# amit154154/HyperscaleES_T2I

Hardware: AMD Instinct MI355X
Metric: ES member-evals/sec (whole node) Sana-Sprint 1.6B pop=64; % HBM/MFMA roofline (higher is better)
Workload: dtype bf16; 1 GPU; sana_sprint_1.6b_onestep_1024px_es_epoch; pop_per_gpu=8, pop_total=8, images_per_member=16, prompts_per_gen=4, batches_per_gen=4, resolution_px=1024, egg_rank=1, lora_r=2, lora_alpha=8, theta_D=1515456, antithetic=True, promptnorm=True, reward=PickScore(CLIP-H/14)+CLIP-B/32, parallelism=member-shard x1 (S all-gather)

## Files before the change

### hyperscalees_t2i_amd/_lib.py

```python
from __future__ import annotations

import ctypes as C
import hashlib
import os
import re
from pathlib import Path

_PKG = Path(__file__).resolve().parent
LIB_PATH = _PKG / "_build" / "libeggroll.so"
HEADER = _PKG.parent / "include" / "eggroll.h"
from .build_ext import SOURCES

SOURCE_FILES = [_PKG / "csrc" / n for n in SOURCES] + sorted((_PKG / "csrc").glob("*.h")) + [HEADER]

i32, i64, u32, u64, f32 = C.c_int32, C.c_int64, C.c_uint32, C.c_uint64, C.c_float
vp = C.c_void_p

SIGNATURES = {
    "eggroll_version": (C.c_char_p, []),
    "eggroll_last_error": (C.c_char_p, []),
    "eggroll_noise_factors": (C.c_int, [u64, i64, i64, i64, i64, vp, vp]),
    "eggroll_philox_words": (C.c_int, [u64, i64, i64, vp, vp]),
    "eggroll_perturb": (C.c_int, [vp, vp, i64, i64, vp, vp, i64, i64, i32, i32, i32, i64, i64, f32, vp, i64, vp]),
    "eggroll_perturb_seeded": (C.c_int, [u64, vp, vp, vp, i64, i64, i32, i32, i32, i64, i64, f32, vp, i64, vp]),
# ... 5 lines not shown
    "eggroll_update_seeded": (C.c_int, [u64, vp, vp, vp, i32, i32, vp, vp, i64, i64, i32, f32, f32, f32, vp, vp, vp]),
    "eggroll_lora_linear_pop": (C.c_int, [vp, i64, vp, i64, vp, vp, i64, i64, i64, i32, f32, i64, i64, i64, i64, vp,
                                          i64, vp, vp]),
    "eggroll_lora_gemm": (C.c_int, [vp, i64, vp, i64, vp, vp, vp, i64, i64, i32, f32, i64, i64, i64, i64, vp, i64, vp]),
    "eggroll_lora_gemm_sel": (C.c_int, [vp, i64, vp, i64, vp, vp, vp, i64, i64, i32, f32, i64, i64, i64, i64, vp, i64,
                                        i32, vp]),
    "eggroll_lora_linear_pop_sel": (C.c_int, [vp, i64, vp, i64, vp, vp, i64, i64, i64, i32, f32, i64, i64, i64, i64,
                                              vp, i64, vp, i32, vp]),
    "eggroll_lora_workspace_bytes": (i64, [i64, i64, i32, i64]),
    "eggroll_lora_project": (C.c_int, [vp, i64, vp, i64, i64, i32, i64, i64, i64, vp, vp]),
    "eggroll_lora_project_multi": (C.c_int, [vp, i64, vp, i64, vp, i32, i32, i64, i64, i64, vp, vp]),
    "eggroll_lora_delta_f32": (C.c_int, [vp, i64, vp, i64, vp, i64, i32, f32, i64, i64, i64, i64, vp, i64, vp]),
    "eggroll_dwconv_nhwc": (C.c_int, [vp, vp, vp, i64, i64, i64, i64, i32, i32, i32, vp, vp]),
    "eggroll_rownorm": (C.c_int, [vp, i64, i64, f32, i32, vp, vp, vp, vp, i64, i64, i32, vp, vp, vp]),
    "eggroll_gated_residual": (C.c_int, [vp, vp, vp, i64, i64, i64, i64, vp]),
    "eggroll_rownorm_ex": (C.c_int, [vp, i32, i64, i64, f32, i32, vp, vp, vp, vp, i64, i32, i64, i32, vp, i32, vp, i32,
                                     vp, vp]),
    "eggroll_subpixel_shortcut_f32": (C.c_int, [vp, vp, vp, vp, vp, i64, i64, i64, i64, i64, vp]),
    "eggroll_gated_residual_f32": (C.c_int, [vp, vp, vp, i32, i64, i64, i64, i64, vp, vp]),
    "eggroll_scm_step": (C.c_int, [vp, i64, vp, i32, vp, i64, i64, f32, f32, f32, f32, f32, f32, f32, f32, f32, i32, vp,
                                   vp, vp, vp]),
    "eggroll_resid_layernorm": (C.c_int, [vp, i64, vp, i64, i64, i64, f32, vp, vp, vp, vp]),
    "eggroll_dwconv_pw_nhwc": (C.c_int, [vp, vp, vp, i64, i64, i64, i64, i32, vp, vp]),
    "eggroll_dwconv_nhwc_sel": (C.c_int, [vp, vp, vp, i64, i64, i64, i64, i32, i32, i32, vp, i32, vp]),
    "eggroll_qk_norm_rope": (C.c_int, [vp, i64, i64, i32, i32, f32, vp, vp, vp, i64, vp]),
    "eggroll_qk_norm_rope_kv": (C.c_int, [vp, i64, i64, i32, i32, f32, vp, vp, vp, i64, vp, vp, i64, i64, i64, i64, vp, i64, vp, vp]),
    "eggroll_qk_l2norm_kv": (C.c_int, [vp, i64, vp, i64, vp, i64, i64, i32, i32, f32, vp, vp, vp, i64, i64, i64, i64, vp]),
    "eggroll_group_norm_workspace_bytes": (C.c_int64, [i64, i64, i32, i32]),
    "eggroll_group_norm_nhwc": (C.c_int, [vp, i64, i64, i32, i32, f32, vp, vp, i32, vp, vp, vp]),
    "eggroll_flash_attention": (C.c_int, [vp, i64, i64, vp, i64, i64, vp, i64, i64, i64, i64, i64, i64, i64, f32, vp, i64, i64, vp]),
    "eggroll_flash_attention_sel": (C.c_int, [vp, i64, i64, vp, i64, i64, vp, i64, i64, i64, i64, i64, i64, i64, f32, vp, i64, i64, i32, vp]),
    "eggroll_dwconv_nhwc_ex": (C.c_int, [vp, vp, vp, i64, i64, i64, i64, i32, i32, i32, vp, i64, i32, vp]),
    "eggroll_dwconv_pw_nhwc_sel": (C.c_int, [vp, vp, vp, i64, i64, i64, i64, i32, vp, i32, vp]),
    "eggroll_upshortcut_add": (C.c_int, [vp, vp, i64, i64, i64, i64, i64, vp]),
    "eggroll_subpixel_shortcut": (C.c_int, [vp, vp, vp, vp, i64, i64, i64, i64, i64, vp]),
    "eggroll_bias_act": (C.c_int, [vp, vp, i64, i64, i32, vp]),
    "eggroll_conv3x3_nhwc": (C.c_int, [vp, vp, vp, i64, i64, i64, i64, i64, i32, i32, vp, vp]),
    "eggroll_conv_nhwc": (C.c_int, [vp, vp, vp, i64, i64, i64, i64, i64, i32, i32, i32, vp, vp]),
    "eggroll_conv3x3_rmsnorm_nhwc": (C.c_int, [vp, vp, vp, i64, i64, i64, i64, i64, i32, C.c_float, vp, vp, vp, vp,
                                               vp]),
    "eggroll_conv_nhwc_sel": (C.c_int, [vp, vp, vp, i64, i64, i64, i64, i64, i32, i32, i32, vp, i32, vp]),
    "eggroll_conv2x2_subpixel_nhwc": (C.c_int, [vp, vp, vp, vp, i32, i64, i64, i64, i64, i64, vp, vp, vp]),
    "eggroll_conv3x3_rmsnorm_nhwc_sel": (C.c_int, [vp, vp, vp, i64, i64, i64, i64, i64, i32, C.c_float, vp, vp, vp,
                                                   vp, i32, vp]),
    "eggroll_dcae_head": (C.c_int, [vp, i64, i64, i64, i64, f32, vp, vp, vp, vp, vp, vp]),
    "eggroll_linear_attention_workspace_bytes": (i64, [i64, i64, i64]),
    "eggroll_linear_attention": (C.c_int, [vp, vp, vp, i64, i64, i64, i64, i64, i32, vp, i64, vp, vp]),
    "eggroll_lora_expand": (C.c_int, [vp, vp, i64, i64, i32, f32, i64, i64, i64, vp, i64, vp]),
    "eggroll_lora_linear_pop_epi": (C.c_int, [vp, i64, vp, i64, vp, vp, i64, i64, i64, i32, f32, i64, i64, i64, i64,
                                              vp, i64, vp, i32, vp, i64, vp, i64, i64, vp]),
    "eggroll_lora_linear_pop_epi_sel": (C.c_int, [vp, i64, vp, i64, vp, vp, i64, i64, i64, i32, f32, i64, i64, i64,
                                                  i64, vp, i64, vp, i32, vp, i64, vp, i64, i64, i32, vp]),
    "eggroll_lora_gemm_epi_sel": (C.c_int, [vp, i64, vp, i64, vp, vp, vp, i64, i64, i32, f32, i64, i64, i64, i64,
                                            vp, i64, i32, vp, i64, vp, i64, i64, i32, vp]),
    "eggroll_cross_attention": (C.c_int, [vp, i64, vp, vp, i64, vp, vp, i64, i64, i64, i64, i64, i64, f32, vp, i64,
                                         vp]),
    "eggroll_cross_attention_sel": (C.c_int, [vp, i64, vp, vp, i64, vp, vp, i64, i64, i64, i64, i64, i64, f32, vp,
                                             i64, i32, vp]),
    "eggroll_clip_preprocess": (C.c_int, [vp, i64, i64, i64, i64, i64, i64, i64, i32, vp, vp, i32, i32, i64, i64,
                                          i64, vp, vp, vp, vp, vp]),
    "eggroll_clip_preprocess_u8": (C.c_int, [vp, i64, i64, i64, i64, i64, i64, i64, vp, vp, i32, i32, i64, i64, i64,
                                             vp, vp, vp, vp, vp]),
    "eggroll_images_to_u8": (C.c_int, [vp, i64, i64, i64, i64, i64, i64, i64, i32, vp, vp]),
    "eggroll_relbias_attention": (C.c_int, [vp, i64, vp, i64, vp, i64, vp, i64, vp, i64, i64, i64, i64, f32, vp, i64,
                                            vp]),
    "eggroll_softcap_attention": (C.c_int, [vp, i64, vp, i64, vp, i64, vp, i64, i64, i64, i64, i64, f32, f32, vp, i64,
# ... 73 lines not shown
```

### hyperscalees_t2i_amd/csrc/eggroll_nhwc.hip

```cpp
#include "frag.h"

namespace eggroll {

constexpr int DW_CS = 32;
constexpr int DW_TW = 32;
constexpr int DW_TH = 8;
constexpr int DW_ORDER_AUTO = 0;
#ifndef EGG_DW5_DOT2
#define EGG_DW5_DOT2 0
#endif

template <int KS, bool PRE_SILU, bool GLU, bool PW = false>
__global__ __launch_bounds__(256) void k_dwconv_nhwc(const unsigned short* __restrict__ in,
                                                     const unsigned short* __restrict__ wt,
                                                     const unsigned short* __restrict__ bias,
                                                     int H, int W, int Cin, int xtiles, int bands, int cslices,
                                                     unsigned short* __restrict__ out,
                                                     const unsigned short* __restrict__ pw = nullptr, int ord = 0,
                                                     int ldo = 0) {
    static_assert(!PW || (!GLU && DW_CS == 32 && DW_TH * DW_TW == 256), "PW: one 32-channel group per block");
    constexpr int PLANES = GLU ? 2 : 1;
    constexpr int HALO = KS / 2;
    constexpr int TR = DW_TH + KS - 1, TC = DW_TW + KS - 1;
    constexpr int PIXB = DW_CS * 2;
    constexpr int IN_BYTES = PLANES * TR * TC * PIXB;
    constexpr int PW_BYTES = PW ? DW_TH * DW_TW * 64 : 0;
    __shared__ __attribute__((aligned(16))) char lds[IN_BYTES + PW_BYTES];
    char* const pwt = lds + IN_BYTES;
    auto swz = [](uint32_t L) { return L ^ ((L >> 3) & 32u); };
    const int Cout = GLU ? Cin / 2 : Cin;
    const int64_t ldo_ = ldo > 0 ? ldo : Cout;
    const int tid = threadIdx.x;
    int bid = xcd_remap(blockIdx.x, gridDim.x);
    int cs, xt, band;
    if (ord == 0) {
        cs = bid % cslices;
        bid /= cslices;
        xt = bid % xtiles;
        bid /= xtiles;
        band = bid % bands;
        bid /= bands;
    } else {
        const int cp = (cslices & 1) ? 1 : 2, chi = cslices / cp;
        const int clo = bid % cp;
        bid /= cp;
        band = bid % bands;
        bid /= bands;
        xt = bid % xtiles;
        bid /= xtiles;
        cs = (bid % chi) * cp + clo;
        bid /= chi;
    }
    const int b = bid;
    const int y0 = band * DW_TH, x0 = xt * DW_TW, c0 = cs * DW_CS;
    const char* img = reinterpret_cast<const char*>(in + (int64_t)b * H * W * Cin);
    const uint32_t cin2 = (uint32_t)Cin * 2, rowb = (uint32_t)W * cin2;
    constexpr uint32_t OOR = 0x80000000u;
    const int rp = __builtin_amdgcn_readfirstlane(tid >> 7);
    const int mc = (tid >> 2) & 31, ch = tid & 3;
    const uint32_t mvoff = x0 + mc < W ? (uint32_t)(x0 + mc) * cin2 + (uint32_t)(c0 * 2 + ch * 16) : OOR;
    constexpr int MPASS = PLANES * TR / 2;
    static_assert(TR % 2 == 0, "row pairs");
    u16x8m v[MPASS];
#pragma unroll
    for (int p = 0; p < MPASS; ++p) {
        const int pl = (2 * p) / TR, ty = (2 * p) % TR + rp;
        const int gy = y0 + ty - HALO;
        const bool ok = gy >= 0 && gy < H;
        const __amdgpu_buffer_rsrc_t rs = __builtin_amdgcn_make_buffer_rsrc(
            (void*)(img + (int64_t)(ok ? gy : 0) * rowb + pl * Cout * 2), (short)0, ok ? (int)rowb : 0, 0x00020000);
        v[p] = __builtin_bit_cast(u16x8m, __builtin_amdgcn_raw_buffer_load_b128(rs, mvoff, 0, 0));
    }
    constexpr int HC = 2 * HALO, HUNITS = PLANES * TR * HC * 4, HPER = (HUNITS + 255) / 256;
    const __amdgpu_buffer_rsrc_t rimg = __builtin_amdgcn_make_buffer_rsrc((void*)img, (short)0, (int)(H * rowb),
                                                                          0x00020000);
    u16x8m hv[HPER];
    uint32_t hlds[HPER];
#pragma unroll
    for (int k = 0; k < HPER; ++k) {
        const int u = tid + k * 256;
        const int hch = u & 3, hcol = (u >> 2) % HC, row = (u >> 2) / HC;
        const int pl = row / TR, ty = row - pl * TR;
        const int tx = hcol < HALO ? hcol : hcol + DW_TW;
        const int gy = y0 + ty - HALO, gx = x0 + tx - HALO;
        const bool ok = u < HUNITS && gy >= 0 && gy < H && gx >= 0 && gx < W;
        const uint32_t off = ok ? (uint32_t)(gy * W + gx) * cin2 + (uint32_t)((pl * Cout + c0) * 2 + hch * 16) : OOR;
        hv[k] = __builtin_bit_cast(u16x8m, __builtin_amdgcn_raw_buffer_load_b128(rimg, off, 0, 0));
        hlds[k] = u < HUNITS ? (uint32_t)(((pl * TR + ty) * TC + tx) * 64 + hch * 16) : 0xffffffffu;
    }
    auto pre = [](u16x8m& x) {
        if (PRE_SILU) {
#pragma unroll
            for (int i = 0; i < 8; ++i) x[i] = f2b(silu(b2f(x[i])));
        }
    };
    const uint32_t mlds = (uint32_t)((rp * TC + HALO + mc) * 64 + ch * 16);
#pragma unroll
    for (int p = 0; p < MPASS; ++p) {
        pre(v[p]);
        *reinterpret_cast<u16x8m*>(lds + mlds + (2 * p) * TC * 64) = v[p];
    }
#pragma unroll
    for (int k = 0; k < HPER; ++k) {
        if (hlds[k] != 0xffffffffu) {
            pre(hv[k]);
            *reinterpret_cast<u16x8m*>(lds + hlds[k]) = hv[k];
        }
    }
    __syncthreads();
    const int q = tid & 7, xs = tid >> 3;
    const int x = x0 + xs;
    const int cq = c0 + q * 4;
    auto rd = [&](int pl, int ty, int tx, float (&f)[4]) {
        const u16x4m v = *reinterpret_cast<const u16x4m*>(lds + ((pl * TR + ty) * TC + tx) * PIXB + q * 8);
#pragma unroll
        for (int i = 0; i < 4; ++i) f[i] = b2f(v[i]);
    };
    const int64_t obase = (int64_t)b * H * W * ldo_;
    const __amdgpu_buffer_rsrc_t rout = __builtin_amdgcn_make_buffer_rsrc(
        (void*)(out + obase), (short)0, (int)((int64_t)H * W * ldo_ * 2), 0x00020000);
    float res[DW_TH][4];
#pragma unroll 1
    for (int pl = 0; pl < PLANES; ++pl) {
        constexpr bool DOT2 = KS == 5 && EGG_DW5_DOT2;
        float w[DOT2 ? 1 : KS * KS][4], bs[4];
        uint32_t wd[DOT2 ? KS * KS : 1][4];
        const __amdgpu_buffer_rsrc_t rw = __builtin_amdgcn_make_buffer_rsrc(
            (void*)(wt + pl * Cout), (short)0, (int)(KS * KS * cin2), 0x00020000);
#pragma unroll
        for (int t = 0; t < KS * KS; ++t) {
            const u16x4m wv = __builtin_bit_cast(u16x4m, __builtin_amdgcn_raw_buffer_load_b64(rw, (uint32_t)cq * 2,
                                                                                            t * (int)cin2, 0));
            if constexpr (DOT2) {
#pragma unroll
                for (int i = 0; i < 4; ++i) wd[t][i] = (i & 1) ? ((uint32_t)wv[i] << 16) : (uint32_t)wv[i];
            } else {
#pragma unroll
                for (int i = 0; i < 4; ++i) w[t][i] = b2f(wv[i]);
            }
        }
        if (bias) {
            const __amdgpu_buffer_rsrc_t rb = __builtin_amdgcn_make_buffer_rsrc((void*)(bias + pl * Cout), (short)0,
                                                                                (int)cin2, 0x00020000);
            const u16x4m bv = __builtin_bit_cast(u16x4m, __builtin_amdgcn_raw_buffer_load_b64(rb, (uint32_t)cq * 2, 0, 0));
#pragma unroll
            for (int i = 0; i < 4; ++i) bs[i] = b2f(bv[i]);
        } else {
#pragma unroll
            for (int i = 0; i < 4; ++i) bs[i] = 0.0f;
        }
        auto emit = [&](int oy, const float (&acc)[4]) {
            if constexpr (PW) {
                u16x4m o;
#pragma unroll
                for (int i = 0; i < 4; ++i) o[i] = f2b(acc[i]);
                *reinterpret_cast<u16x4m*>(pwt + swz((uint32_t)((oy * DW_TW + xs) * 64 + q * 8))) = o;
            } else if (pl == 0 && GLU) {
#pragma unroll
                for (int i = 0; i < 4; ++i) res[oy][i] = acc[i];
            } else {
                const int y = y0 + oy;
                u16x4m o;
#pragma unroll
                for (int i = 0; i < 4; ++i) o[i] = f2b(GLU ? res[oy][i] * silu(acc[i]) : acc[i]);
                const uint32_t px = (uint32_t)(y * W + x) * (uint32_t)ldo_ * 2;
                const bool ok = y < H && x < W;
                __builtin_amdgcn_raw_buffer_store_b64(__builtin_bit_cast(u32x2m, o), rout,
                                                      ok ? px + (uint32_t)cq * 2 : OOR, 0, 0);
                if (ldo_ > Cout && cs == cslices - 1 && Cout + q * 4 < ldo_)
                    __builtin_amdgcn_raw_buffer_store_b64(u32x2m{0u, 0u}, rout,
                                                          ok ? px + (uint32_t)(Cout + q * 4) * 2 : OOR, 0, 0);
            }
        };
        if constexpr (KS == 3) {
            float win[KS][KS][4];
#pragma unroll
            for (int r = 0; r < KS - 1; ++r)
#pragma unroll
                for (int dx = 0; dx < KS; ++dx) rd(pl, r, xs + dx, win[r][dx]);
#pragma unroll
            for (int oy = 0; oy < DW_TH; ++oy) {
#pragma unroll
                for (int dx = 0; dx < KS; ++dx) rd(pl, oy + KS - 1, xs + dx, win[KS - 1][dx]);
                float acc[4];
#pragma unroll
                for (int i = 0; i < 4; ++i) acc[i] = bs[i];
#pragma unroll
                for (int dy = 0; dy < KS; ++dy)
#pragma unroll
                    for (int dx = 0; dx < KS; ++dx)
#pragma unroll
                        for (int i = 0; i < 4; ++i) acc[i] += win[dy][dx][i] * w[dy * KS + dx][i];
#pragma unroll
                for (int r = 0; r < KS - 1; ++r)
#pragma unroll
                    for (int dx = 0; dx < KS; ++dx)
#pragma unroll
                        for (int i = 0; i < 4; ++i) win[r][dx][i] = win[r + 1][dx][i];
                emit(oy, acc);
            }
        } else {
#pragma unroll 1
            for (int oy = 0; oy < DW_TH; ++oy) {
                float acc[4];
#pragma unroll
                for (int i = 0; i < 4; ++i) acc[i] = bs[i];
#pragma unroll
                for (int dy = 0; dy < KS; ++dy)
#pragma unroll
                    for (int dx = 0; dx < KS; ++dx) {
                        if constexpr (DOT2) {
                            typedef __attribute__((ext_vector_type(2))) __bf16 dw_bf2;
                            const u32x2m v = *reinterpret_cast<const u32x2m*>(
                                lds + ((pl * TR + oy + dy) * TC + xs + dx) * PIXB + q * 8);
                            const uint32_t xw[2] = {v.x, v.y};
#pragma unroll
                            for (int i = 0; i < 4; ++i)
                                acc[i] = __builtin_amdgcn_fdot2_f32_bf16(__builtin_bit_cast(dw_bf2, xw[i >> 1]),
                                                                         __builtin_bit_cast(dw_bf2, wd[dy * KS + dx][i]),
                                                                         acc[i], false);
                        } else {
                            float tap[4];
                            rd(pl, oy + dy, xs + dx, tap);
#pragma unroll
                            for (int i = 0; i < 4; ++i) acc[i] += tap[i] * w[dy * KS + dx][i];
                        }
                    }
                emit(oy, acc);
            }
        }
    }
    if constexpr (PW) {
        __syncthreads();
        const int lane = tid & 63, wv = tid >> 6, r16 = lane & 15, g4 = lane >> 4;
        const unsigned short* pg = pw + (int64_t)cs * (DW_CS * DW_CS);
        la_bf16x8 bo[2];
#pragma unroll
        for (int j = 0; j < 2; ++j)
            bo[j] = *reinterpret_cast<const la_bf16x8*>(pg + (16 * j + r16) * DW_CS + 8 * g4);
#pragma unroll
        for (int f = 0; f < 4; ++f) {
            const int p = wv * 64 + 16 * f + r16;
            const la_bf16x8 a = *reinterpret_cast<const la_bf16x8*>(pwt + swz((uint32_t)(p * 64 + g4 * 16)));
            const int y = y0 + (p >> 5), xx = x0 + (p & 31);
#pragma unroll
            for (int j = 0; j < 2; ++j) {
                const la_f32x4 d = __builtin_amdgcn_mfma_f32_16x16x32_bf16(bo[j], a, la_f32x4{0.f, 0.f, 0.f, 0.f}, 0, 0, 0);
                u16x4m o;
#pragma unroll
                for (int e = 0; e < 4; ++e) o[e] = f2b(d[e]);
                const uint32_t off = y < H && xx < W ? ((uint32_t)(y * W + xx) * Cout + c0 + 16 * j + 4 * g4) * 2 : OOR;
                __builtin_amdgcn_raw_buffer_store_b64(__builtin_bit_cast(u32x2m, o), rout, off, 0, 0);
            }
        }
    }
}

__global__ __launch_bounds__(256) void k_upshortcut_add(unsigned short* __restrict__ y, const unsigned short* __restrict__ x,
                                                        int H, int W, int Cin, int Cout, int rep, int pix_total) {
    const int groups = Cout >> 3;
    const int t = blockIdx.x * blockDim.x + threadIdx.x;
    const int pix = t / groups;
    if (pix >= pix_total) return;
    const int c0 = (t - pix * groups) << 3;
    const int W2 = 2 * W, HW4 = 4 * H * W;
// ... 226 lines not shown
            for (int tap = 0; tap < 9; ++tap)
                abase[r][tap] = (uint32_t)hd_slot(slot(j8, wave * 2 + r + tap / 3) * HD_TC + n + tap % 3, g);
        __syncthreads();
        hd_f32x4 acc[2] = {hd_f32x4{0.f, 0.f, 0.f, 0.f}, hd_f32x4{0.f, 0.f, 0.f, 0.f}};
#pragma unroll
        for (int s = 0; s < 36; ++s) {
            const int tap = s >> 2, cq = s & 3;
            const hd_bf16x8 bf = *reinterpret_cast<const hd_bf16x8*>(wl + wrow + tap * HD_C + cq * 32);
#pragma unroll
            for (int r = 0; r < 2; ++r) {
                const hd_bf16x8 af = *reinterpret_cast<const hd_bf16x8*>(tile + (abase[r][tap] ^ (uint32_t)(cq << 6)));
                acc[r] = __builtin_amdgcn_mfma_f32_16x16x32_bf16(af, bf, acc[r], 0, 0, 0);
            }
        }
        if (n < 3) {
#pragma unroll
            for (int r = 0; r < 2; ++r) {
                const int yy = y0 + wave * 2 + r;
#pragma unroll
                for (int e = 0; e < 4; ++e) {
                    const int xx = x0 + 4 * g + e;
                    if (yy < H && xx < W) y[(((int64_t)b * H + yy) * W + xx) * 3 + n] = f2b(acc[r][e] + bias);
                }
            }
        }
        j8 = slot(j8, HD_TH);
    }
}

}

using namespace eggroll;

static int dw_order(int kernel) { return kernel == 0 ? DW_ORDER_AUTO : kernel - 1; }

template <bool PW>
static void dw_launch(int ks, bool pre_silu, bool glu, int64_t nblk, hipStream_t st, const void* in, const void* w_t,
                      const void* bias, int64_t H, int64_t W, int64_t C, int64_t xtiles, int64_t bands, int64_t cslices,
                      void* out, const void* pw, int kernel, int64_t ldo) {
    dispatch_int(ks, std::integer_sequence<int, 3, 5>{}, [&](auto KS) {
        dispatch_int(pre_silu, Flag01{}, [&](auto PS) {
            dispatch_int(glu, Flag01{}, [&](auto GL) {
                if constexpr (!PW || (!decltype(PS)::value && !decltype(GL)::value))
                    hipLaunchKernelGGL((k_dwconv_nhwc<decltype(KS)::value, decltype(PS)::value, decltype(GL)::value, PW>),
                                       dim3((unsigned)nblk), dim3(256), 0, st, (const unsigned short*)in,
                                       (const unsigned short*)w_t, (const unsigned short*)bias, (int)H, (int)W, (int)C,
                                       (int)xtiles, (int)bands, (int)cslices, (unsigned short*)out,
                                       (const unsigned short*)pw, dw_order(kernel), (int)ldo);
            });
        });
    });
}

extern "C" int eggroll_dwconv_nhwc(const void* in, const void* w_t, const void* bias, int64_t B, int64_t H, int64_t W,
                                   int64_t C, int32_t ks, int32_t pre_silu, int32_t glu, void* out, void* stream) {
    return eggroll_dwconv_nhwc_sel(in, w_t, bias, B, H, W, C, ks, pre_silu, glu, out, 0, stream);
}

extern "C" int eggroll_dwconv_nhwc_sel(const void* in, const void* w_t, const void* bias, int64_t B, int64_t H,
                                       int64_t W, int64_t C, int32_t ks, int32_t pre_silu, int32_t glu, void* out,
                                       int32_t kernel, void* stream) {
    return eggroll_dwconv_nhwc_ex(in, w_t, bias, B, H, W, C, ks, pre_silu, glu, out, glu ? C / 2 : C, kernel, stream);
}

extern "C" int eggroll_dwconv_nhwc_ex(const void* in, const void* w_t, const void* bias, int64_t B, int64_t H,
                                      int64_t W, int64_t C, int32_t ks, int32_t pre_silu, int32_t glu, void* out,
                                      int64_t ldo, int32_t kernel, void* stream) {
    EGG_CHECK_ARG(kernel >= 0 && kernel <= 2, "dwconv: kernel must be 0 (auto), 1 (channel-fastest) or 2 (column "
                  "sweep) (got %d)", kernel);
    EGG_CHECK_ARG(B >= 0 && H > 0 && W > 0 && C > 0, "dwconv: bad sizes");
    const int64_t cout = glu ? C / 2 : C;
    EGG_CHECK_ARG((!glu || C % 2 == 0) && cout % DW_CS == 0, "dwconv: output channels must be a multiple of %d", DW_CS);
    EGG_CHECK_ARG(ldo >= cout && ldo - cout <= DW_CS && ldo % 8 == 0,
                  "dwconv: output row stride %lld must be in [%lld, %lld] and a multiple of 8", (long long)ldo,
                  (long long)cout, (long long)(cout + DW_CS));
    EGG_CHECK_ARG(ks == 3 || ks == 5, "dwconv: ks=%d unsupported (3, 5)", ks);
    EGG_CHECK_ARG(((uintptr_t)in & 15) == 0 && ((uintptr_t)w_t & 15) == 0 && ((uintptr_t)out & 15) == 0,
                  "dwconv: pointers must be 16-byte aligned");
    EGG_CHECK_ARG(H * W * C < (1ll << 30) && H * W * ldo < (1ll << 30), "dwconv: image too large (< 2 GiB per image)");
    if (B == 0) return EGGROLL_OK;
    EGG_CHECK_ARG(in && w_t && out, "dwconv: NULL pointer");
    const int64_t bands = (H + DW_TH - 1) / DW_TH, xtiles = (W + DW_TW - 1) / DW_TW, cslices = cout / DW_CS;
    const int64_t nblk = B * bands * xtiles * cslices;
    EGG_CHECK_ARG(nblk < (1ll << 31), "dwconv: grid too large");
    dw_launch<false>(ks, pre_silu != 0, glu != 0, nblk, as_stream(stream), in, w_t, bias, H, W, C, xtiles, bands, cslices,
                     out, nullptr, kernel, ldo);
    EGG_CHECK_LAUNCH("dwconv_nhwc");
    return EGGROLL_OK;
}

extern "C" int eggroll_dwconv_pw_nhwc(const void* in, const void* w_t, const void* pw, int64_t B, int64_t H, int64_t W,
                                      int64_t C, int32_t ks, void* out, void* stream) {
    return eggroll_dwconv_pw_nhwc_sel(in, w_t, pw, B, H, W, C, ks, out, 0, stream);
}

extern "C" int eggroll_dwconv_pw_nhwc_sel(const void* in, const void* w_t, const void* pw, int64_t B, int64_t H,
                                          int64_t W, int64_t C, int32_t ks, void* out, int32_t kernel, void* stream) {
    EGG_CHECK_ARG(kernel >= 0 && kernel <= 2, "dwconv_pw: kernel must be 0 (auto), 1 or 2 (got %d)", kernel);
    EGG_CHECK_ARG(B >= 0 && H > 0 && W > 0 && C > 0 && C % DW_CS == 0, "dwconv_pw: C must be a multiple of %d", DW_CS);
    EGG_CHECK_ARG(ks == 3 || ks == 5, "dwconv_pw: ks=%d unsupported (3, 5)", ks);
    EGG_CHECK_ARG(((uintptr_t)in & 15) == 0 && ((uintptr_t)w_t & 15) == 0 && ((uintptr_t)out & 15) == 0 &&
                      ((uintptr_t)pw & 15) == 0,
                  "dwconv_pw: pointers must be 16-byte aligned");
    EGG_CHECK_ARG(H * W * C < (1ll << 30), "dwconv_pw: image too large (< 2 GiB per image)");
    if (B == 0) return EGGROLL_OK;
    EGG_CHECK_ARG(in && w_t && pw && out && out != in, "dwconv_pw: NULL or aliased pointer");
    const int64_t bands = (H + DW_TH - 1) / DW_TH, xtiles = (W + DW_TW - 1) / DW_TW, cslices = C / DW_CS;
    const int64_t nblk = B * bands * xtiles * cslices;
    EGG_CHECK_ARG(nblk < (1ll << 31), "dwconv_pw: grid too large");
    dw_launch<true>(ks, false, false, nblk, as_stream(stream), in, w_t, nullptr, H, W, C, xtiles, bands, cslices, out, pw,
                    kernel, 0);
    EGG_CHECK_LAUNCH("dwconv_pw_nhwc");
    return EGGROLL_OK;
}

extern "C" int eggroll_upshortcut_add(void* y, const void* x, int64_t B, int64_t H, int64_t W, int64_t Cin,
                                      int64_t Cout, void* stream) {
    EGG_CHECK_ARG(B >= 0 && H > 0 && W > 0 && Cin > 0 && Cout > 0 && (4 * Cout) % Cin == 0 && Cout % 8 == 0,
                  "upshortcut: bad sizes");
    EGG_CHECK_ARG(B * 4 * H * W * Cout < (1ll << 31) && B * H * W * Cin < (1ll << 31), "upshortcut: tensor too large");
    if (B == 0) return EGGROLL_OK;
    EGG_CHECK_ARG(x && y, "upshortcut: NULL pointer");
    const int64_t pix = B * 4 * H * W;
    const int64_t threads = pix * (Cout / 8);
    hipLaunchKernelGGL(k_upshortcut_add, dim3((unsigned)((threads + 255) / 256)), dim3(256), 0, as_stream(stream),
                       (unsigned short*)y, (const unsigned short*)x, (int)H, (int)W, (int)Cin, (int)Cout,
                       (int)(4 * Cout / Cin), (int)pix);
    EGG_CHECK_LAUNCH("upshortcut_add");
    return EGGROLL_OK;
}

// ... 77 lines not shown
```

### hyperscalees_t2i_amd/kernels.py

```python
from __future__ import annotations

import math
from dataclasses import dataclass, field
from typing import Dict, List, Optional, Sequence, Tuple

import numpy as np
import torch

from . import _lib

CHUNK = 1024


def _dev(t: torch.Tensor, what: str, dtype=None, contiguous: bool = True) -> torch.Tensor:
    if not isinstance(t, torch.Tensor) or t.device.type != "cuda":
        raise _lib.EggrollError(f"{what}: expected a ROCm device tensor, got "
                                f"{getattr(t, 'device', type(t))} (no CPU fallback)")
    if dtype is not None and t.dtype != dtype:
        raise _lib.EggrollError(f"{what}: expected dtype {dtype}, got {t.dtype}")
    if contiguous and not t.is_contiguous():
        raise _lib.EggrollError(f"{what}: tensor must be contiguous")
    return t


# ... 485 lines not shown
                    x["tflops"] = x["flops"] / (x["total_ms"] * 1e9)
                    x["mfma_frac"] = x["tflops"] / 2500.0
                else:
                    x.pop("flops")
            top = sorted(d["shapes"].items(), key=lambda kv: -kv[1]["total_ms"])[:4]
            d["shapes"] = {k: {kk: round(vv, 3) for kk, vv in v.items()} for k, v in top}
        return out




def dwconv_nhwc(x: torch.Tensor, w_t: torch.Tensor, bias: Optional[torch.Tensor], ks: int, pre_silu: bool,
                glu: bool, out: Optional[torch.Tensor] = None, kernel: int = 0, ldo: int = 0) -> torch.Tensor:
    _dev(x, "dwconv(x)", torch.bfloat16)
    _dev(w_t, "dwconv(w_t)", torch.bfloat16)
    B, H, W, C = x.shape
    if w_t.shape != (ks * ks, C):
        raise ValueError(f"w_t {tuple(w_t.shape)} != ({ks * ks}, {C})")
    if bias is not None:
        _dev(bias, "dwconv(bias)", torch.bfloat16)
    co = C // 2 if glu else C
    ldo = ldo or co
    if out is None:
        out = torch.empty((B, H, W, ldo), dtype=torch.bfloat16, device=x.device)
    elif out.shape != (B, H, W, ldo) or not out.is_contiguous():
        raise ValueError(f"dwconv(out) {tuple(out.shape)} != ({B}, {H}, {W}, {ldo}) contiguous")
    e0 = OpTimer.begin()
    _lib.call("eggroll_dwconv_nhwc_ex", x.data_ptr(), w_t.data_ptr(), _p(bias), B, H, W, C, ks, int(pre_silu),
              int(glu), out.data_ptr(), ldo, int(kernel), _stream(x.device))
    OpTimer.end(e0, f"dwconv_nhwc<{ks},{int(pre_silu)},{int(glu)}>", 2.0 * B * H * W * (C + co), f"{B}x{H}x{W}x{C}")
    return out


def dwconv_pw_nhwc(x: torch.Tensor, w_t: torch.Tensor, pw: torch.Tensor, ks: int,
                   out: Optional[torch.Tensor] = None, kernel: int = 0) -> torch.Tensor:
    _dev(x, "dwconv_pw(x)", torch.bfloat16)
    _dev(w_t, "dwconv_pw(w_t)", torch.bfloat16)
    _dev(pw, "dwconv_pw(pw)", torch.bfloat16)
    x, pw = x.contiguous(), pw.contiguous()
    B, H, W, C = x.shape
    if w_t.shape != (ks * ks, C) or pw.shape != (C // 32, 32, 32) or C % 32:
        raise ValueError(f"dwconv_pw: w_t {tuple(w_t.shape)} / pw {tuple(pw.shape)} do not match C={C}, ks={ks}")
    if out is None:
        out = torch.empty_like(x)
    e0 = OpTimer.begin()
    _lib.call("eggroll_dwconv_pw_nhwc_sel", x.data_ptr(), w_t.data_ptr(), pw.data_ptr(), B, H, W, C, ks,
              out.data_ptr(), int(kernel), _stream(x.device))
    OpTimer.end(e0, f"dwconv_pw_nhwc<{ks}>", 4.0 * B * H * W * C, f"{B}x{H}x{W}x{C}")
    return out


def _row_ptr(t: Optional[torch.Tensor], what: str, C: int, allow_f32: bool = False):
    if t is None:
        return None, 0
    ok = (torch.bfloat16, torch.float32) if allow_f32 else (torch.bfloat16,)
    if t.device.type != "cuda" or t.dtype not in ok or t.stride(-1) != 1:
        raise _lib.EggrollError(f"{what}: expected a {'bf16 / fp32' if allow_f32 else 'bf16'} device view with "
                                f"unit inner stride")
    stride = t.stride(0) if t.dim() > 1 and t.shape[0] > 1 else C
    return t.data_ptr(), stride


ACT = {None: 0, "none": 0, "relu": 1, "silu": 2}


def rownorm(x: torch.Tensor, eps: float, layer: bool = False, w: Optional[torch.Tensor] = None,
# ... 658 lines not shown
```

### include/eggroll.h

```cpp
#ifndef EGGROLL_H_
#define EGGROLL_H_

#include <stdint.h>

#ifdef __cplusplus
extern "C" {
#endif

#define EGGROLL_OK 0
#define EGGROLL_ERR_ARG (-1)
#define EGGROLL_ERR_LAUNCH (-2)
#define EGGROLL_ERR_UNSUPPORTED (-3)

typedef struct eggroll_mat {
    int64_t rows;
    int64_t cols;
    int64_t theta_off;
    int64_t factor_off;
    int64_t chunk_off;
    int64_t reserved;
} eggroll_mat_t;

typedef struct eggroll_tile {
    int32_t mat;
// ... 71 lines not shown
                      int64_t K, void* Y, int64_t ldy, void* stream);
int eggroll_lora_gemm_sel(const void* X, int64_t ldx, const void* W, int64_t ldw, const void* bias,
                          const float* T, const float* theta_pop, int64_t ld_theta, int64_t offB,
                          int32_t r, float scale, int64_t rows_per_member, int64_t M, int64_t N,
                          int64_t K, void* Y, int64_t ldy, int32_t kernel, void* stream);
int eggroll_lora_linear_pop_sel(const void* X, int64_t ldx, const void* W, int64_t ldw,
                                const void* bias, const float* theta_pop, int64_t ld_theta,
                                int64_t offA, int64_t offB, int32_t r, float scale,
                                int64_t rows_per_member, int64_t M, int64_t N, int64_t K,
                                void* Y, int64_t ldy, float* T_ws, int32_t kernel, void* stream);
int eggroll_lora_project(const void* X, int64_t ldx, const float* theta_pop, int64_t ld_theta,
                         int64_t offA, int32_t r, int64_t rows_per_member, int64_t M, int64_t K,
                         float* T, void* stream);
int eggroll_lora_project_multi(const void* X, int64_t ldx, const float* theta_pop, int64_t ld_theta,
                               const int64_t* offA_host, int32_t n_lin, int32_t r, int64_t rows_per_member,
                               int64_t M, int64_t K, float* T, void* stream);
int eggroll_lora_expand(const float* T, const float* theta_pop, int64_t ld_theta, int64_t offB,
                        int32_t r, float scale, int64_t rows_per_member, int64_t M, int64_t N,
                        void* Y, int64_t ldy, void* stream);
int eggroll_lora_delta_f32(const float* x, int64_t ldx, const float* A, int64_t lda_member, const float* B,
                           int64_t ldb_member, int32_t r, float scale, int64_t rows_per_member, int64_t M,
                           int64_t N, int64_t K, float* y, int64_t ldy, void* stream);

int eggroll_dwconv_nhwc(const void* in, const void* w_t, const void* bias, int64_t B, int64_t H,
                        int64_t W, int64_t C, int32_t ks, int32_t pre_silu, int32_t glu, void* out,
                        void* stream);
int eggroll_dwconv_pw_nhwc(const void* in, const void* w_t, const void* pw, int64_t B, int64_t H,
                           int64_t W, int64_t C, int32_t ks, void* out, void* stream);
int eggroll_dwconv_nhwc_sel(const void* in, const void* w_t, const void* bias, int64_t B, int64_t H,
                            int64_t W, int64_t C, int32_t ks, int32_t pre_silu, int32_t glu, void* out,
                            int32_t kernel, void* stream);
int eggroll_dwconv_pw_nhwc_sel(const void* in, const void* w_t, const void* pw, int64_t B, int64_t H,
                               int64_t W, int64_t C, int32_t ks, void* out, int32_t kernel, void* stream);
int eggroll_dwconv_nhwc_ex(const void* in, const void* w_t, const void* bias, int64_t B, int64_t H,
                           int64_t W, int64_t C, int32_t ks, int32_t pre_silu, int32_t glu, void* out,
                           int64_t ldo, int32_t kernel, void* stream);

int eggroll_rownorm(const void* x, int64_t rows, int64_t C, float eps, int32_t layer, const void* w,
                    const void* b, const void* mscale, const void* mshift, int64_t mstride,
                    int64_t rows_per_group, int32_t act, const void* res, void* out, void* stream);
int eggroll_gated_residual(void* x, const void* y, const void* gate, int64_t gstride, int64_t rows,
                           int64_t C, int64_t rows_per_group, void* stream);
int eggroll_qk_norm_rope(void* x, int64_t ldx, int64_t rows, int32_t heads, int32_t head_dim, float eps,
                         const void* w, const float* cos_tab, const float* sin_tab, int64_t tab_rows, void* stream);
int eggroll_qk_norm_rope_kv(void* x, int64_t ldx, int64_t rows, int32_t heads, int32_t head_dim, float eps,
                            const void* w, const float* cos_tab, const float* sin_tab, int64_t tab_rows,
                            const float* hscale, void* out, int64_t out_bs, int64_t out_ld, int64_t rows_per_seq,
                            int64_t row0, const void* vin, int64_t ldv, void* vout, void* stream);
int eggroll_qk_l2norm_kv(void* q, int64_t ldq, void* k, int64_t ldk, const void* v, int64_t ldv, int64_t rows,
                         int32_t heads, int32_t head_dim, float eps, const float* qscale, void* kout, void* vout,
                         int64_t out_bs, int64_t out_ld, int64_t rows_per_seq, int64_t row0, void* stream);
int eggroll_rownorm_ex(const void* x, int32_t x_f32, int64_t rows, int64_t C, float eps, int32_t layer,
                       const void* w, const void* b, const void* mscale, const void* mshift, int64_t mstride,
                       int32_t mod_f32, int64_t rows_per_group, int32_t act, const void* res, int32_t res_f32,
                       void* out, int32_t out_f32, void* shadow, void* stream);
int eggroll_gated_residual_f32(float* x, const void* y, const void* gate, int32_t gate_f32, int64_t gstride,
                               int64_t rows, int64_t C, int64_t rows_per_group, void* shadow, void* stream);
int eggroll_scm_step(const float* x, int64_t x_member_stride, const void* eps, int32_t eps_f32, const float* noise,
                     int64_t members, int64_t n, float in_scale, float coef_m, float coef_eps, float cos_t,
                     float sin_t, float cos_n, float sin_n_sd, float in_scale_next, float out_scale,
                     int32_t round_dtype, float* x_next, float* m_next, float* x0_out, void* stream);
int eggroll_resid_layernorm(float* h, int64_t ldh, const void* y, int64_t ldy, int64_t rows, int64_t C,
                            float eps, const void* w, const void* b, void* out, void* stream);
int eggroll_upshortcut_add(void* y, const void* x, int64_t B, int64_t H, int64_t W, int64_t Cin,
                           int64_t Cout, void* stream);

// ... 93 lines not shown
```

Baseline: 5.875 member-evals/s.

## Compute 5x5 depthwise conv via MFMA diagonal-weight matmuls in dwconv+pointwise kernel

Adds an MFMA form of the NHWC depthwise conv kernel. Each tap is done as a 16x16x16 bf16 MFMA with a block-diagonal weight fragment. Weights and bias are preloaded into registers, GLU planes are staged one at a time through a smaller shared buffer with an XOR swizzle, and the depthwise outputs stay in registers until they are written for the pointwise stage. By default this applies only to the fused dwconv+pointwise ks=5 path, where it also sets waves_per_eu=5. The aim is to move the VALU FMA work onto matrix units and cut LDS use. The cost is many wasted MFMA lanes, since most of each diagonal fragment is zero, plus extra barriers.

```diff
diff --git a/hyperscalees_t2i_amd/_lib.py b/hyperscalees_t2i_amd/_lib.py
--- a/hyperscalees_t2i_amd/_lib.py
+++ b/hyperscalees_t2i_amd/_lib.py
@@ -61,6 +61,7 @@
     "eggroll_flash_attention_sel": (C.c_int, [vp, i64, i64, vp, i64, i64, vp, i64, i64, i64, i64, i64, i64, i64, f32, vp, i64, i64, i32, vp]),
     "eggroll_dwconv_nhwc_ex": (C.c_int, [vp, vp, vp, i64, i64, i64, i64, i32, i32, i32, vp, i64, i32, vp]),
     "eggroll_dwconv_pw_nhwc_sel": (C.c_int, [vp, vp, vp, i64, i64, i64, i64, i32, vp, i32, vp]),
+    "eggroll_dwconv_default_form": (C.c_int, [i32, i32, i32, i32]),
     "eggroll_upshortcut_add": (C.c_int, [vp, vp, i64, i64, i64, i64, i64, vp]),
     "eggroll_subpixel_shortcut": (C.c_int, [vp, vp, vp, vp, i64, i64, i64, i64, i64, vp]),
     "eggroll_bias_act": (C.c_int, [vp, vp, i64, i64, i32, vp]),
diff --git a/hyperscalees_t2i_amd/csrc/eggroll_nhwc.hip b/hyperscalees_t2i_amd/csrc/eggroll_nhwc.hip
--- a/hyperscalees_t2i_amd/csrc/eggroll_nhwc.hip
+++ b/hyperscalees_t2i_amd/csrc/eggroll_nhwc.hip
@@ -6,12 +6,13 @@
 constexpr int DW_TW = 32;
 constexpr int DW_TH = 8;
 constexpr int DW_ORDER_AUTO = 0;
+typedef __attribute__((ext_vector_type(4))) unsigned int u32x4m;
 #ifndef EGG_DW5_DOT2
 #define EGG_DW5_DOT2 0
 #endif
 
-template <int KS, bool PRE_SILU, bool GLU, bool PW = false>
-__global__ __launch_bounds__(256) void k_dwconv_nhwc(const unsigned short* __restrict__ in,
+template <int KS, bool PRE_SILU, bool GLU, bool PW = false, bool MF = false>
+__global__ __launch_bounds__(256) __attribute__((amdgpu_waves_per_eu(MF && PW && KS == 5 ? 5 : 1))) void k_dwconv_nhwc(const unsigned short* __restrict__ in,
                                                      const unsigned short* __restrict__ wt,
                                                      const unsigned short* __restrict__ bias,
                                                      int H, int W, int Cin, int xtiles, int bands, int cslices,
@@ -23,11 +24,14 @@
     constexpr int HALO = KS / 2;
     constexpr int TR = DW_TH + KS - 1, TC = DW_TW + KS - 1;
     constexpr int PIXB = DW_CS * 2;
-    constexpr int IN_BYTES = PLANES * TR * TC * PIXB;
+    constexpr int LPLANES = MF ? 1 : PLANES;
+    constexpr int IN_BYTES = LPLANES * TR * TC * PIXB;
     constexpr int PW_BYTES = PW ? DW_TH * DW_TW * 64 : 0;
-    __shared__ __attribute__((aligned(16))) char lds[IN_BYTES + PW_BYTES];
-    char* const pwt = lds + IN_BYTES;
+    constexpr int LDS_BYTES = MF ? (IN_BYTES > PW_BYTES ? IN_BYTES : PW_BYTES) : IN_BYTES + PW_BYTES;
+    __shared__ __attribute__((aligned(16))) char lds[LDS_BYTES];
+    char* const pwt = MF ? lds : lds + IN_BYTES;
     auto swz = [](uint32_t L) { return L ^ ((L >> 3) & 32u); };
+    auto tsw = [](int tx) -> uint32_t { return MF ? (uint32_t)((tx >> 2) & 3) * 16u : 0u; };
     const int Cout = GLU ? Cin / 2 : Cin;
     const int64_t ldo_ = ldo > 0 ? ldo : Cout;
     const int tid = threadIdx.x;
@@ -76,6 +80,7 @@
                                                                           0x00020000);
     u16x8m hv[HPER];
     uint32_t hlds[HPER];
+    int hpl[HPER];
 #pragma unroll
     for (int k = 0; k < HPER; ++k) {
         const int u = tid + k * 256;
@@ -86,7 +91,33 @@
         const bool ok = u < HUNITS && gy >= 0 && gy < H && gx >= 0 && gx < W;
         const uint32_t off = ok ? (uint32_t)(gy * W + gx) * cin2 + (uint32_t)((pl * Cout + c0) * 2 + hch * 16) : OOR;
         hv[k] = __builtin_bit_cast(u16x8m, __builtin_amdgcn_raw_buffer_load_b128(rimg, off, 0, 0));
-        hlds[k] = u < HUNITS ? (uint32_t)(((pl * TR + ty) * TC + tx) * 64 + hch * 16) : 0xffffffffu;
+        hlds[k] = u < HUNITS ? (uint32_t)((((MF ? 0 : pl) * TR + ty) * TC + tx) * 64 + hch * 16) ^ tsw(tx) : 0xffffffffu;
+        hpl[k] = pl;
+    }
+    const int q = MF ? ((tid >> 6) & 1) * 4 + ((tid & 63) >> 4) : tid & 7;
+    const int xs = MF ? (tid >> 7) * 16 + (tid & 15) : tid >> 3;
+    const int cq = c0 + q * 4;
+    constexpr int NM = KS * KS;
+    uint32_t wraw[MF ? PLANES : 1][MF ? NM : 1];
+    u32x2m braw[MF ? PLANES : 1];
+    if constexpr (MF) {
+        const int m = tid & 15, chh = (tid >> 6) & 1;
+#pragma unroll
+        for (int pl = 0; pl < PLANES; ++pl) {
+            const __amdgpu_buffer_rsrc_t rw = __builtin_amdgcn_make_buffer_rsrc(
+                (void*)(wt + pl * Cout), (short)0, (int)(KS * KS * cin2), 0x00020000);
+#pragma unroll
+            for (int j = 0; j < NM; ++j) {
+                wraw[pl][j] = (uint32_t)__builtin_amdgcn_raw_buffer_load_b16(rw, (uint32_t)(c0 + chh * 16 + m) * 2,
+                                                                             j * (int)cin2, 0) & 0xffffu;
+            }
+            braw[pl] = u32x2m{0u, 0u};
+            if (bias) {
+                const __amdgpu_buffer_rsrc_t rb = __builtin_amdgcn_make_buffer_rsrc(
+                    (void*)(bias + pl * Cout), (short)0, (int)cin2, 0x00020000);
+                braw[pl] = __builtin_amdgcn_raw_buffer_load_b64(rb, (uint32_t)cq * 2, 0, 0);
+            }
+        }
     }
     auto pre = [](u16x8m& x) {
         if (PRE_SILU) {
@@ -94,23 +125,28 @@
             for (int i = 0; i < 8; ++i) x[i] = f2b(silu(b2f(x[i])));
         }
     };
-    const uint32_t mlds = (uint32_t)((rp * TC + HALO + mc) * 64 + ch * 16);
-#pragma unroll
-    for (int p = 0; p < MPASS; ++p) {
-        pre(v[p]);
-        *reinterpret_cast<u16x8m*>(lds + mlds + (2 * p) * TC * 64) = v[p];
-    }
-#pragma unroll
-    for (int k = 0; k < HPER; ++k) {
-        if (hlds[k] != 0xffffffffu) {
-            pre(hv[k]);
-            *reinterpret_cast<u16x8m*>(lds + hlds[k]) = hv[k];
-        }
-    }
-    __syncthreads();
-    const int q = tid & 7, xs = tid >> 3;
+    const uint32_t mlds = (uint32_t)((rp * TC + HALO + mc) * 64 + ch * 16) ^ tsw(HALO + mc);
+    auto stage = [&](int ps) {
+#pragma unroll
+        for (int p = 0; p < MPASS; ++p) {
+            const int pl = (2 * p) / TR;
+            if (ps >= 0 && pl != ps) continue;
+            pre(v[p]);
+            *reinterpret_cast<u16x8m*>(lds + mlds + (2 * p - (ps >= 0 ? pl * TR : 0)) * TC * 64) = v[p];
+        }
+#pragma unroll
+        for (int k = 0; k < HPER; ++k) {
+            if (hlds[k] != 0xffffffffu && (ps < 0 || hpl[k] == ps)) {
+                pre(hv[k]);
+                *reinterpret_cast<u16x8m*>(lds + hlds[k]) = hv[k];
+            }
+        }
+    };
+    if constexpr (!MF) {
+        stage(-1);
+        __syncthreads();
+    }
     const int x = x0 + xs;
-    const int cq = c0 + q * 4;
     auto rd = [&](int pl, int ty, int tx, float (&f)[4]) {
         const u16x4m v = *reinterpret_cast<const u16x4m*>(lds + ((pl * TR + ty) * TC + tx) * PIXB + q * 8);
 #pragma unroll
@@ -120,15 +156,38 @@
     const __amdgpu_buffer_rsrc_t rout = __builtin_amdgcn_make_buffer_rsrc(
         (void*)(out + obase), (short)0, (int)((int64_t)H * W * ldo_ * 2), 0x00020000);
     float res[DW_TH][4];
-#pragma unroll 1
+    u32x2m pwr[PW && MF ? DW_TH : 1];
+    constexpr int PLU = MF ? PLANES : 1;
+#pragma unroll PLU
     for (int pl = 0; pl < PLANES; ++pl) {
-        constexpr bool DOT2 = KS == 5 && EGG_DW5_DOT2;
-        float w[DOT2 ? 1 : KS * KS][4], bs[4];
+        if constexpr (MF) {
+            if (pl > 0) __syncthreads();
+            stage(pl);
+            __syncthreads();
+        }
+        constexpr bool DOT2 = KS == 5 && EGG_DW5_DOT2 && !MF;
+        constexpr int NT = MF ? 0 : KS * KS;
+        float w[DOT2 || MF ? 1 : KS * KS][4], bs[4];
         uint32_t wd[DOT2 ? KS * KS : 1][4];
         const __amdgpu_buffer_rsrc_t rw = __builtin_amdgcn_make_buffer_rsrc(
             (void*)(wt + pl * Cout), (short)0, (int)(KS * KS * cin2), 0x00020000);
-#pragma unroll
-        for (int t = 0; t < KS * KS; ++t) {
+        u32x2m wf[MF ? NM : 1];
+        uint32_t pa[MF ? KS : 1];
+        if constexpr (MF) {
+            const int lane = tid & 63, m = lane & 15, c = lane >> 4;
+            const int chh = (tid >> 6) & 1, xb = (tid >> 7) * 16 + m;
+            const bool diag = (m >> 2) == c;
+#pragma unroll
+            for (int j = 0; j < NM; ++j) {
+                const uint32_t wv = diag ? wraw[pl][j] << ((m & 1) * 16) : 0u;
+                wf[j] = (m & 2) ? u32x2m{0u, wv} : u32x2m{wv, 0u};
+            }
+#pragma unroll
+            for (int dx = 0; dx < KS; ++dx)
+                pa[dx] = ((uint32_t)((xb + dx) * 64 + chh * 32 + (c >> 1) * 16) ^ tsw(xb + dx)) + (uint32_t)(c & 1) * 8;
+        }
+#pragma unroll
+        for (int t = 0; t < NT; ++t) {
             const u16x4m wv = __builtin_bit_cast(u16x4m, __builtin_amdgcn_raw_buffer_load_b64(rw, (uint32_t)cq * 2,
                                                                                             t * (int)cin2, 0));
             if constexpr (DOT2) {
@@ -139,7 +198,11 @@
                 for (int i = 0; i < 4; ++i) w[t][i] = b2f(wv[i]);
             }
         }
-        if (bias) {
+        if constexpr (MF) {
+            const u16x4m bv = __builtin_bit_cast(u16x4m, braw[pl]);
+#pragma unroll
+            for (int i = 0; i < 4; ++i) bs[i] = b2f(bv[i]);
+        } else if (bias) {
             const __amdgpu_buffer_rsrc_t rb = __builtin_amdgcn_make_buffer_rsrc((void*)(bias + pl * Cout), (short)0,
                                                                                 (int)cin2, 0x00020000);
             const u16x4m bv = __builtin_bit_cast(u16x4m, __builtin_amdgcn_raw_buffer_load_b64(rb, (uint32_t)cq * 2, 0, 0));
@@ -154,7 +217,10 @@
                 u16x4m o;
 #pragma unroll
                 for (int i = 0; i < 4; ++i) o[i] = f2b(acc[i]);
-                *reinterpret_cast<u16x4m*>(pwt + swz((uint32_t)((oy * DW_TW + xs) * 64 + q * 8))) = o;
+                if constexpr (MF)
+                    pwr[oy] = __builtin_bit_cast(u32x2m, o);
+                else
+                    *reinterpret_cast<u16x4m*>(pwt + swz((uint32_t)((oy * DW_TW + xs) * 64 + q * 8))) = o;
             } else if (pl == 0 && GLU) {
 #pragma unroll
                 for (int i = 0; i < 4; ++i) res[oy][i] = acc[i];
@@ -172,7 +238,33 @@
                                                           ok ? px + (uint32_t)(Cout + q * 4) * 2 : OOR, 0, 0);
             }
         };
-        if constexpr (KS == 3) {
+        if constexpr (MF) {
+#pragma unroll
+            for (int oy = 0; oy < DW_TH; ++oy) {
+                la_f32x4 d = {bs[0], bs[1], bs[2], bs[3]};
+#pragma unroll
+                for (int j = 0; GLU && j < NM; ++j) {
+                    const la_s4 px = *reinterpret_cast<const la_s4*>(lds + pa[j % KS] + (oy + j / KS) * TC * 64);
+                    d = __builtin_amdgcn_mfma_f32_16x16x16bf16_1k(__builtin_bit_cast(la_s4, wf[j]), px, d, 0, 0, 0);
+                }
+#pragma unroll
+                for (int dy = 0; !GLU && dy < KS; ++dy) {
+                    la_f32x4 p[KS];
+#pragma unroll
+                    for (int dx = 0; dx < KS; ++dx) {
+                        const la_s4 px = *reinterpret_cast<const la_s4*>(lds + pa[dx] + (oy + dy) * TC * 64);
+                        p[dx] = __builtin_amdgcn_mfma_f32_16x16x16bf16_1k(__builtin_bit_cast(la_s4, wf[dy * KS + dx]), px,
+                                                                          la_f32x4{0.f, 0.f, 0.f, 0.f}, 0, 0, 0);
+                    }
+#pragma unroll
+                    for (int dx = 0; dx < KS; ++dx) d += p[dx];
+                    __builtin_amdgcn_sched_barrier(0x3f4);
+                }
+                if constexpr (!GLU) __builtin_amdgcn_sched_barrier(0);
+                const float acc[4] = {d[0], d[1], d[2], d[3]};
+                emit(oy, acc);
+            }
+        } else if constexpr (KS == 3) {
             float win[KS][KS][4];
 #pragma unroll
             for (int r = 0; r < KS - 1; ++r)
@@ -231,6 +323,12 @@
         }
     }
     if constexpr (PW) {
+        if constexpr (MF) {
+            __syncthreads();
+#pragma unroll
+            for (int oy = 0; oy < DW_TH; ++oy)
+                *reinterpret_cast<u32x2m*>(pwt + swz((uint32_t)((oy * DW_TW + xs) * 64 + q * 8))) = pwr[oy];
+        }
         __syncthreads();
         const int lane = tid & 63, wv = tid >> 6, r16 = lane & 15, g4 = lane >> 4;
         const unsigned short* pg = pw + (int64_t)cs * (DW_CS * DW_CS);
@@ -523,24 +621,38 @@
 
 using namespace eggroll;
 
-static int dw_order(int kernel) { return kernel == 0 ? DW_ORDER_AUTO : kernel - 1; }
+static int dw_order(int kernel) { return kernel == 1 || kernel == 2 ? kernel - 1 : DW_ORDER_AUTO; }
+
+static bool dw_default_mfma(int ks, bool pre_silu, bool glu, bool pw) {
+    (void)pre_silu;
+    (void)glu;
+    return pw && ks == 5;
+}
 
 template <bool PW>
 static void dw_launch(int ks, bool pre_silu, bool glu, int64_t nblk, hipStream_t st, const void* in, const void* w_t,
                       const void* bias, int64_t H, int64_t W, int64_t C, int64_t xtiles, int64_t bands, int64_t cslices,
                       void* out, const void* pw, int kernel, int64_t ldo) {
+    const bool mf = kernel == 4 || (kernel != 3 && dw_default_mfma(ks, pre_silu, glu, PW));
     dispatch_int(ks, std::integer_sequence<int, 3, 5>{}, [&](auto KS) {
         dispatch_int(pre_silu, Flag01{}, [&](auto PS) {
             dispatch_int(glu, Flag01{}, [&](auto GL) {
-                if constexpr (!PW || (!decltype(PS)::value && !decltype(GL)::value))
-                    hipLaunchKernelGGL((k_dwconv_nhwc<decltype(KS)::value, decltype(PS)::value, decltype(GL)::value, PW>),
-                                       dim3((unsigned)nblk), dim3(256), 0, st, (const unsigned short*)in,
-                                       (const unsigned short*)w_t, (const unsigned short*)bias, (int)H, (int)W, (int)C,
-                                       (int)xtiles, (int)bands, (int)cslices, (unsigned short*)out,
-                                       (const unsigned short*)pw, dw_order(kernel), (int)ldo);
+                dispatch_int(mf, Flag01{}, [&](auto MF) {
+                    if constexpr (!PW || (!decltype(PS)::value && !decltype(GL)::value))
+                        hipLaunchKernelGGL((k_dwconv_nhwc<decltype(KS)::value, decltype(PS)::value, decltype(GL)::value,
+                                                          PW, decltype(MF)::value>),
+                                           dim3((unsigned)nblk), dim3(256), 0, st, (const unsigned short*)in,
+                                           (const unsigned short*)w_t, (const unsigned short*)bias, (int)H, (int)W, (int)C,
+                                           (int)xtiles, (int)bands, (int)cslices, (unsigned short*)out,
+                                           (const unsigned short*)pw, dw_order(kernel), (int)ldo);
+                });
             });
         });
     });
+}
+
+extern "C" int eggroll_dwconv_default_form(int32_t ks, int32_t pre_silu, int32_t glu, int32_t pw) {
+    return dw_default_mfma(ks, !pw && pre_silu, !pw && glu, pw != 0) ? 4 : 3;
 }
 
 extern "C" int eggroll_dwconv_nhwc(const void* in, const void* w_t, const void* bias, int64_t B, int64_t H, int64_t W,
@@ -557,8 +669,8 @@
 extern "C" int eggroll_dwconv_nhwc_ex(const void* in, const void* w_t, const void* bias, int64_t B, int64_t H,
                                       int64_t W, int64_t C, int32_t ks, int32_t pre_silu, int32_t glu, void* out,
                                       int64_t ldo, int32_t kernel, void* stream) {
-    EGG_CHECK_ARG(kernel >= 0 && kernel <= 2, "dwconv: kernel must be 0 (auto), 1 (channel-fastest) or 2 (column "
-                  "sweep) (got %d)", kernel);
+    EGG_CHECK_ARG(kernel >= 0 && kernel <= 4, "dwconv: kernel must be 0 (auto), 1 (channel-fastest), 2 (column "
+                  "sweep), 3 (VALU form) or 4 (MFMA form) (got %d)", kernel);
     EGG_CHECK_ARG(B >= 0 && H > 0 && W > 0 && C > 0, "dwconv: bad sizes");
     const int64_t cout = glu ? C / 2 : C;
     EGG_CHECK_ARG((!glu || C % 2 == 0) && cout % DW_CS == 0, "dwconv: output channels must be a multiple of %d", DW_CS);
@@ -587,7 +699,8 @@
 
 extern "C" int eggroll_dwconv_pw_nhwc_sel(const void* in, const void* w_t, const void* pw, int64_t B, int64_t H,
                                           int64_t W, int64_t C, int32_t ks, void* out, int32_t kernel, void* stream) {
-    EGG_CHECK_ARG(kernel >= 0 && kernel <= 2, "dwconv_pw: kernel must be 0 (auto), 1 or 2 (got %d)", kernel);
+    EGG_CHECK_ARG(kernel >= 0 && kernel <= 4, "dwconv_pw: kernel must be 0 (auto), 1, 2 (block orders), 3 (VALU form) "
+                  "or 4 (MFMA form) (got %d)", kernel);
     EGG_CHECK_ARG(B >= 0 && H > 0 && W > 0 && C > 0 && C % DW_CS == 0, "dwconv_pw: C must be a multiple of %d", DW_CS);
     EGG_CHECK_ARG(ks == 3 || ks == 5, "dwconv_pw: ks=%d unsupported (3, 5)", ks);
     EGG_CHECK_ARG(((uintptr_t)in & 15) == 0 && ((uintptr_t)w_t & 15) == 0 && ((uintptr_t)out & 15) == 0 &&
diff --git a/hyperscalees_t2i_amd/kernels.py b/hyperscalees_t2i_amd/kernels.py
--- a/hyperscalees_t2i_amd/kernels.py
+++ b/hyperscalees_t2i_amd/kernels.py
@@ -541,6 +541,10 @@
     return out
 
 
+def dwconv_default_form(ks: int, pre_silu: bool = False, glu: bool = False, pw: bool = False) -> int:
+    return int(_lib.load().eggroll_dwconv_default_form(int(ks), int(pre_silu), int(glu), int(pw)))
+
+
 def dwconv_pw_nhwc(x: torch.Tensor, w_t: torch.Tensor, pw: torch.Tensor, ks: int,
                    out: Optional[torch.Tensor] = None, kernel: int = 0) -> torch.Tensor:
     _dev(x, "dwconv_pw(x)", torch.bfloat16)
diff --git a/include/eggroll.h b/include/eggroll.h
--- a/include/eggroll.h
+++ b/include/eggroll.h
@@ -127,6 +127,7 @@
                             int32_t kernel, void* stream);
 int eggroll_dwconv_pw_nhwc_sel(const void* in, const void* w_t, const void* pw, int64_t B, int64_t H,
                                int64_t W, int64_t C, int32_t ks, void* out, int32_t kernel, void* stream);
+int eggroll_dwconv_default_form(int32_t ks, int32_t pre_silu, int32_t glu, int32_t pw);
 int eggroll_dwconv_nhwc_ex(const void* in, const void* w_t, const void* bias, int64_t B, int64_t H,
                            int64_t W, int64_t C, int32_t ks, int32_t pre_silu, int32_t glu, void* out,
                            int64_t ldo, int32_t kernel, void* stream);
```

Result: no change. 5.900 member-evals/s, median of 6 (+0.4%).
